# Adamtaranto/frisk

Measured on AMD Instinct MI355X. Metric: windows/sec (k=1..8, w=5kb, s=1kb), higher is better.
Workload: dtype u8/u4 counts + f64 scores

## Files before the change

frisk_amd/csrc/scan8_kernel.h:

```cpp
#pragma once
#include "scan_kernel.h"
#include "ring_rows.h"

#define FRISK8_ORPH_CAP 24
#define FRISK8_UNROLL1 2
#define FRISK8_SHORT_LANES 6
#define FRISK8_PRIO 3
#define FRISK8_RING_PAD 16
#define FRISK8_SLOTS 8

enum { M8_NPLACED = 1,
       M8_PMASK = 3,
       M8_TSUM = 6,
       M8_SAFE = 7 };

template <int KMAX, int BITS, int LOGN, int NT, bool SIDE = false>
struct Lds8 {
    static constexpr uint32_t small = 0;
    static constexpr uint32_t small_bytes = 2736;
    static constexpr uint32_t orphans = small + small_bytes;
    static constexpr uint32_t NL = 1u << (2 * (KMAX - 3));
    static constexpr uint32_t pre = (orphans + FRISK8_ORPH_CAP * 2 + 15) / 16 * 16;
    static constexpr uint32_t side = pre + NL * 12;
    static constexpr uint32_t logtab = side + (SIDE ? 256 : 0);
    static constexpr uint32_t rctab = logtab + uint32_t(LOGN) * 16;
    static constexpr uint32_t misc = rctab + (SIDE ? 256 * 16 : 16 * (BITS == 4 ? 16 : 8));
    static constexpr uint32_t t8 = (misc + 2 * FRISK8_SLOTS * 4 + uint32_t(NT / 64) * 3 * 8 + 15) / 16 * 16;
    static constexpr uint32_t t8_bytes = (1u << (2 * KMAX)) * BITS / 8;
    static constexpr uint32_t total = t8 + t8_bytes;
    static constexpr uint32_t granules = (total + 1279) / 1280;
};

template <int N, int DEG>
__device__ inline double log_tab_n(double x, const double2* tab) {
    const int k = __builtin_amdgcn_frexp_exp(x);
    const double m = __builtin_amdgcn_frexp_mant(x);
    const uint32_t off = (uint32_t(__double2hiint(m)) >> ((N == 128 ? 13 : (N == 64 ? 14 : 15)) - 4)) & (uint32_t(N - 1) << 4);
    const double2 e = *reinterpret_cast<const double2*>(reinterpret_cast<const char*>(tab) + off);
    const double r = __builtin_fma(m, e.x, -1.0);
    double p = (DEG & 1) ? 1.0 / DEG : -1.0 / DEG;
#pragma unroll
    for (int d = DEG - 1; d >= 2; --d) p = __builtin_fma(r, p, (d & 1) ? 1.0 / d : -1.0 / d);
    return __builtin_fma(double(k), 0.69314718055994530942, e.y) + __builtin_fma(r * r, p, r);
}

template <int CTRL>
__device__ inline uint32_t dpp_addu(uint32_t x) {
    return x + uint32_t(__builtin_amdgcn_update_dpp(0, int(x), CTRL, 0xF, 0xF, false));
}
__device__ inline uint32_t wave_sum_u32(uint32_t x) {
    x = dpp_addu<0xB1>(x); x = dpp_addu<0x4E>(x); x = dpp_addu<0x141>(x); x = dpp_addu<0x140>(x);
    return __builtin_amdgcn_readlane(int(x), 0) + __builtin_amdgcn_readlane(int(x), 16) +
           __builtin_amdgcn_readlane(int(x), 32) + __builtin_amdgcn_readlane(int(x), 48);
}

__global__ void scan8_decide_kernel(const unsigned int* __restrict__ counts, unsigned int n_sampled, double side_share, int side_ok,
                                    unsigned int* __restrict__ verdict) {
    const unsigned int handed = counts[0], would = counts[2], scored = counts[3];
    unsigned int form = (double(handed) <= 0.3 * double(n_sampled)) ? 1u : 3u;
    if (form == 1u && side_ok && double(handed + would) > side_share * double(handed + scored)) form = 2u;
    verdict[0] = form; verdict[1] = handed; verdict[2] = would; verdict[3] = scored;
}

template <int KMAX, int NT, int ITS, int BITS, int LOGN, int WPS, bool DEBUG, int ROLE = 0, bool SIDE = false>
__global__ __launch_bounds__(NT, WPS) void scan8_kernel(const ScanParams P) {
    static_assert(KMAX >= 6 && KMAX <= 8, "highest order 6, 7 or 8");
    constexpr int K = KMAX, LVL = KMAX - 3;
    constexpr uint32_t NK = 1u << (2 * K), NL = 1u << (2 * LVL);
    static_assert(BITS == 4 || BITS == 8, "order-8 counters are 4 or 8 bits wide");
    static_assert(LOGN == 32 || LOGN == 64 || LOGN == 128, "logarithm table of 32, 64 or 128 bins");
    constexpr int LOGDEG = LOGN == 128 ? 5 : (LOGN == 64 ? 6 : 7);
    static_assert(ITS + 7 <= 32, "a lane's positions and their max-mers must fit the 32 bases it loads");
    constexpr int NW = NT / 64;
    constexpr int SHW = BITS == 8 ? 2 : 3;
    constexpr uint32_t PERM = (32 / BITS) - 1;
    static_assert(!SIDE || (KMAX == 8 && BITS == 4 && !DEBUG && NT == 256), "the side table exists for the 4-bit form at K = 8");
    using L = Lds8<KMAX, BITS, LOGN, NT, SIDE>;
    constexpr bool CLEAR_ALL = L::t8_bytes / 16 / NT <= uint32_t(ITS);
    constexpr bool FUSED = (KMAX >= 7 && NT >= 256 && NT % 256 == 0);
    constexpr bool PLACE = FUSED && !DEBUG;
    __shared__ __attribute__((aligned(16))) unsigned char lds[L::total];
    const int tid0 = threadIdx.x;
    const int kmin0 = P.kmin;
    uint32_t* t8 = reinterpret_cast<uint32_t*>(lds + L::t8);
    const unsigned char* t8b = lds + L::t8;
    uint32_t* small32 = reinterpret_cast<uint32_t*>(lds + L::small);
    uint16_t* small16 = reinterpret_cast<uint16_t*>(lds + L::small);
    uint16_t* orph = reinterpret_cast<uint16_t*>(lds + L::orphans);
    double* preA = reinterpret_cast<double*>(lds + L::pre);
    uint32_t* preW = reinterpret_cast<uint32_t*>(lds + L::pre + NL * 8);
    uint32_t* side32 = reinterpret_cast<uint32_t*>(lds + L::side);
    const unsigned char* side8 = lds + L::side;
    auto put_pre = [&](uint32_t idx, double A, uint32_t W, uint32_t sd = 0u) __attribute__((always_inline)) {
        if constexpr (SIDE) { preA[idx] = A; preW[idx] = W | (sd << 23); }
        else { preA[idx] = A; preW[idx] = W; }
    };
    auto bump = [&](uint32_t c16, auto sign_c) __attribute__((always_inline)) {
        constexpr int SIGN = decltype(sign_c)::value;
        if (SIDE && ((c16 ^ (c16 >> 8)) & 0xFFu) == 0u) {
            const uint32_t one = 1u << ((c16 & 3u) * 8u);
            if (SIGN > 0) atomicAdd(&side32[(c16 & 0xFFu) >> 2], one); else atomicSub(&side32[(c16 & 0xFFu) >> 2], one);
        } else {
            const uint32_t one = 1u << ((c16 & PERM) * BITS);
            if (SIGN > 0) atomicAdd(&t8[c16 >> SHW], one); else atomicSub(&t8[c16 >> SHW], one);
        }
    };
    uint32_t* misc_base = reinterpret_cast<uint32_t*>(lds + L::misc);
    double* scratch = reinterpret_cast<double*>(lds + L::misc + 2 * FRISK8_SLOTS * 4);
    const double2* logtab = reinterpret_cast<const double2*>(lds + L::logtab);
    double2* rstab = reinterpret_cast<double2*>(lds + L::rctab);
    double* rctab = reinterpret_cast<double*>(lds + L::rctab);

    auto clear_t8 = [&]() {
#pragma unroll
        for (int i = tid0; i < int(L::t8_bytes / 16); i += NT) reinterpret_cast<uint4*>(t8)[i] = make_uint4(0, 0, 0, 0);
        if (SIDE && tid0 < 64) side32[tid0] = 0u;
    };
    auto clear_small = [&]() {
        for (uint32_t i = tid0; i < L::small_bytes / 16; i += NT) reinterpret_cast<uint4*>(small32)[i] = make_uint4(0, 0, 0, 0);
    };
    if (P.in_list != nullptr && *P.in_count == 0u) return;
    if (P.verdict != nullptr && *P.verdict != P.my_form) return;
    __builtin_amdgcn_s_setprio(FRISK8_PRIO);
    clear_t8();
    clear_small();
    if (tid0 < 2 * FRISK8_SLOTS) misc_base[tid0] = 0;
    {
        double2* lt = reinterpret_cast<double2*>(lds + L::logtab);
        for (int i = tid0; i < LOGN; i += NT) lt[i] = reinterpret_cast<const double2*>(LOGN == 128 ? P.log_tab : (LOGN == 64 ? P.log_tab64 : P.log_tab32))[i];
        if constexpr (SIDE) {
            static_assert(!SIDE || NT >= 256, "one thread per entry of the reciprocal table");
            if (tid0 < 256) {
                double r = P.rc_tab[tid0 & 15];
                if (tid0 >= 16) {
                    const double dc = double(tid0);
                    r = __builtin_amdgcn_rcp(dc);
                    r = __builtin_fma(r, __builtin_fma(-dc, r, 1.0), r);
                    r = __builtin_fma(r, __builtin_fma(-dc, r, 1.0), r);
                }
                rstab[tid0] = make_double2(r, 0.0);
            }
        } else if (tid0 < 16) {
            if (BITS == 4) rstab[tid0] = make_double2(P.rc_tab[tid0], 0.0); else rctab[tid0] = P.rc_tab[tid0];
        }
    }
    __syncthreads();

    const int G = gridDim.x;
    int v = blockIdx.x;
    if ((G & 7) == 0) v = (blockIdx.x & 7) * (G >> 3) + (blockIdx.x >> 3);
    const bool listed = P.in_list != nullptr;
    const int64_t chunk = listed ? 1 : P.chunk;
    const int64_t nall = listed ? int64_t(*P.in_count) : (P.c1 - P.c0 + chunk - 1) / chunk;
    const int64_t M = P.sel_mod;
    const int64_t nsample = (nall + M - 1) / M;
    const int64_t nchunks = listed || P.sel_mode == 0 ? nall : (P.sel_mode == 1 ? nsample : nall - nsample);

    ScafDesc d;
    d.cand0 = 0; d.ncand = 0; d.off = 0; d.size = 0; d.kind = 0; d.base0 = 0; d.j0 = 0;
    int dsi = -1;
    uint32_t parity = 0;
    const int slide_pp = P.in_list == nullptr ? P.slide_pp : 0;
    constexpr bool RING = KMAX == 8 && BITS == 4 && !(ROLE & 2);
    char* const ring = RING ? reinterpret_cast<char*>(P.ig_ring) : nullptr;
    const uint32_t slice_off = RING ? uint32_t((size_t(NK) + size_t(blockIdx.x) * (size_t(ITS) * FRISK8_RING_COLS + FRISK8_RING_PAD)) * 8) : 0u;
    bool slide_next = false;
    bool ring_next = false;

    auto window_of = [&](int64_t cand, int64_t& st, int64_t& rep_start, int64_t& rep_stop, int& n, bool& jump) {
        const int64_t j = cand - d.cand0 + d.j0;
        jump = false;
        if (d.kind == 1) { st = 0; n = int(d.size); rep_start = 1; rep_stop = d.size; }
        else {
            st = j * P.inc;
            n = P.w;
            rep_start = st + 1; rep_stop = st + P.w;
            if (st + P.w > d.size) {
                jump = true;
                st = d.size - P.w;
                rep_start = st; rep_stop = d.size;
                if (st < 0) { st += d.size; if (st < 0) st = 0; }
                n = int(d.size - st);
            }
        }
    };
    typedef const __attribute__((address_space(4))) ScanParams* KernargView;
    KernargView Pk = (KernargView)__builtin_amdgcn_kernarg_segment_ptr();
    uint32_t* next_q = reinterpret_cast<uint32_t*>(scratch);
    const bool dealt = Pk->queue != nullptr;
    const uint32_t NQ = dealt ? uint32_t(P.queue_n) : 1u;
    const uint32_t myq = blockIdx.x % NQ;
    uint32_t dry = 0, ahead = 0;
    if (dealt && tid0 == 0) ahead = atomicAdd(&Pk->queue[myq], 1u);
    for (int64_t qs = v;; qs += G) {
        int64_t q = qs;
        asm volatile("" : "+s"(Pk));
        if (dealt) {
            if (tid0 == 0) {
                uint32_t got = 0xFFFFFFFFu;
                while (dry < NQ) {
                    const uint32_t j = (myq + dry) % NQ;
                    const int64_t b = nchunks * j / NQ, len = nchunks * (j + 1) / NQ - b;
                    if (int64_t(ahead) < len) { got = uint32_t(b + ahead); break; }
                    if (++dry < NQ) ahead = atomicAdd(&Pk->queue[(myq + dry) % NQ], 1u);
                }
                *next_q = got;
                if (got != 0xFFFFFFFFu) ahead = atomicAdd(&Pk->queue[(myq + dry) % NQ], 1u);
            }
            __syncthreads();
            const uint32_t got = uint32_t(__builtin_amdgcn_readfirstlane(int(*next_q)));
            __syncthreads();
            if (got == 0xFFFFFFFFu) break;
            q = int64_t(got);
        }
        if (q >= nchunks) break;
        int64_t qq = q;
        if (!listed && P.sel_mode == 1) qq = q * M;
        if (!listed && P.sel_mode == 2) qq = (q / (M - 1)) * M + 1 + q % (M - 1);
        const int64_t cb = listed ? q : P.c0 + qq * chunk;
        const int64_t ce = listed ? q + 1 : ((cb + chunk < P.c1) ? cb + chunk : P.c1);
        for (int64_t ci = cb; ci < ce; ++ci) {
            const int64_t cand = listed ? Pk->in_list[ci] : ci;
            if (cand < d.cand0 || cand >= d.cand0 + d.ncand) {
                int lo = 0, hi = P.n_desc - 1;
                while (lo < hi) {
                    const int mid = (lo + hi + 1) >> 1;
                    if (Pk->descs[mid].cand0 <= cand) lo = mid; else hi = mid - 1;
                }
                d = Pk->descs[lo];
                dsi = lo;
                auto s64 = [](int64_t x) -> int64_t {
                    return int64_t((uint64_t(uint32_t(__builtin_amdgcn_readfirstlane(int(uint64_t(x) >> 32)))) << 32) |
                                   uint32_t(__builtin_amdgcn_readfirstlane(int(uint32_t(uint64_t(x))))));
                };
                d.off = s64(d.off); d.size = s64(d.size); d.cand0 = s64(d.cand0); d.ncand = s64(d.ncand);
                d.base0 = s64(d.base0); d.j0 = s64(d.j0); d.kind = __builtin_amdgcn_readfirstlane(d.kind);
            }
            int tid = tid0, kmin = kmin0;
            asm volatile("" : "+v"(tid), "+s"(kmin));
            asm volatile("" : "+s"(Pk));
            const int lane = tid & 63;
            int64_t st, rep_start, rep_stop;
            int n;
            bool jump = false;
            window_of(cand, st, rep_start, rep_stop, n, jump);
            const int64_t g0 = d.off + (st - d.base0);
            const int64_t row = cand - P.c0;
            const uint32_t ring_base = RING ? uint32_t(uint64_t(st) % uint64_t(ITS * FRISK8_RING_COLS)) : 0u;
            const uint32_t rb_q = ring_base / uint32_t(ITS), rb_r = ring_base - rb_q * uint32_t(ITS);
            const uint32_t lane_col0 = RING ? ring_lane_col(rb_q, uint32_t(tid), 0u) : 0u;
            const uint32_t lane_col1 = RING ? ring_lane_col(rb_q, uint32_t(tid), 1u) : 0u;
            auto ring_uni = [&](int it) __attribute__((always_inline)) -> uint32_t {
                return ring_uni_general<ITS>(slice_off, rb_r, it);
            };
            auto ring_lane = [&](int it) __attribute__((always_inline)) -> uint32_t {
                return ring_lane_general<ITS>(rb_r, it, lane_col0, lane_col1);
            };
            auto ring_mine = [&](int it) __attribute__((always_inline)) -> uint32_t { return ring_uni(it) + ring_lane(it); };
            constexpr bool ROWS = RING && ITS == 20;
            typedef const __attribute__((address_space(1))) char* GlobalBytes;
            typedef const __attribute__((address_space(1))) double* GlobalDouble;
            GlobalBytes row0_base = ROWS ? (GlobalBytes)(ring + slice_off + ring_row0_base_row(0) * FRISK8_RING_ROW_BYTES) : nullptr;
            const uint32_t row0_lane = ROWS ? ring_off_row0(slice_off, rb_q, uint32_t(tid), 0) : 0u;
            const bool sliding = slide_next;
            const bool lane_new = !sliding || !ring_next || tid * ITS + (ITS - 1) >= P.w - (K - 1) - P.inc;
            ring_next = false;
            slide_next = slide_pp > 0 && ci + 1 < ce && d.kind == 0 && !jump && cand + 1 < d.cand0 + d.ncand &&
                         st + int64_t(P.inc) + P.w <= d.size;
            if (n > NT * ITS) {
                if (tid == 0) { const unsigned int slot = atomicAdd(Pk->out_count, 1u); Pk->out_list[slot] = cand; }
                continue;
            }
            uint32_t* misc = misc_base + parity * FRISK8_SLOTS;
            uint32_t* misc_other = misc_base + (parity ^ 1u) * FRISK8_SLOTS;
            parity ^= 1u;

            const int j0 = tid * ITS;
            const int64_t gl = g0 + (j0 < n ? j0 : 0);
            const int64_t wi = gl >> 4, mi = gl >> 5;
            const int shc = 32 - int(gl & 15) * 2, shm = 32 - int(gl & 31);
            const uint32_t w0 = P.codes[wi], w1 = P.codes[wi + 1], w2 = P.codes[wi + 2];
            const uint32_t i0 = P.inv[mi], i1 = P.inv[mi + 1], l0 = P.low[mi], l1 = P.low[mi + 1];
            uint64_t scode = 0, ecode = 0;
            uint32_t sfull = 0, efull = 0;
            if (sliding) {
                const int q0 = tid * slide_pp;
                const int cnt = P.inc - q0;
                const int64_t gs = g0 - P.inc + (cnt > 0 ? q0 : 0);
                const int64_t ge = g0 + (P.w - (K - 1) - P.inc) + (cnt > 0 ? q0 : 0);
                const int64_t swi = gs >> 4, smi = gs >> 5, ewi = ge >> 4, emi = ge >> 5;
                const uint32_t s0 = P.codes[swi], s1 = P.codes[swi + 1], s2 = P.codes[swi + 2], si0 = P.inv[smi], si1 = P.inv[smi + 1];
                const uint32_t e0 = P.codes[ewi], e1 = P.codes[ewi + 1], e2 = P.codes[ewi + 2], ei0 = P.inv[emi], ei1 = P.inv[emi + 1];
                auto funnel = [](uint32_t a, uint32_t b, uint32_t c, int sh) -> uint64_t {
                    return (uint64_t(uint32_t(((uint64_t(a) << 32) | b) >> sh)) << 32) | uint32_t(((uint64_t(b) << 32) | c) >> sh);
                };
                auto starts = [](uint32_t inv32, int cnt_, int pp) -> uint32_t {
                    uint32_t f = ~inv32;
                    f &= f << 1; f &= f << 2;
                    f &= f << (K - 4);
                    const int m = cnt_ < pp ? cnt_ : pp;
                    return m > 0 ? f & uint32_t(0xFFFFFFFF00000000ull >> m) : 0u;
                };
                scode = funnel(s0, s1, s2, 32 - int(gs & 15) * 2);
                ecode = funnel(e0, e1, e2, 32 - int(ge & 15) * 2);
                sfull = starts(uint32_t(((uint64_t(si0) << 32) | si1) >> (32 - int(gs & 31))), cnt, slide_pp);
                efull = starts(uint32_t(((uint64_t(ei0) << 32) | ei1) >> (32 - int(ge & 31))), cnt, slide_pp);
            }
            const uint32_t chi = uint32_t(((uint64_t(w0) << 32) | w1) >> shc);
            const uint32_t clo = uint32_t(((uint64_t(w1) << 32) | w2) >> shc);
            const uint64_t acode = (uint64_t(chi) << 32) | clo;
            const uint32_t ainv = uint32_t(((uint64_t(i0) << 32) | i1) >> shm);
            const uint32_t alow = uint32_t(((uint64_t(l0) << 32) | l1) >> shm);
            auto topbits = [](int k) -> uint32_t {
                k = k < 0 ? 0 : (k > 32 ? 32 : k);
                return uint32_t(0xFFFFFFFF00000000ull >> k);
            };
            constexpr uint32_t MINE = uint32_t(0xFFFFFFFF00000000ull >> ITS);
            const int nleft = n - j0;
            const uint32_t actm = topbits(nleft) & MINE;
            const uint32_t vld = ~ainv;
            uint32_t fullm = vld;
            fullm &= fullm << 1; fullm &= fullm << 2;
            fullm &= fullm << (K - 4);
            fullm &= topbits(nleft - (K - 1)) & MINE;
            auto code_at = [&](int it) -> uint32_t { return uint32_t(acode >> (64 - 2 * K - 2 * it)) & (NK - 1u); };
            {
                uint32_t cAll = 0, cGC = 0, nvalid = 0;
                auto gc_plane = [&]() -> uint32_t {
                    auto squeeze = [](uint32_t w) -> uint32_t {
                        uint32_t x = (w >> 1) & 0x55555555u;
                        x = (x | (x >> 1)) & 0x33333333u;
                        x = (x | (x >> 2)) & 0x0F0F0F0Fu;
                        x = (x | (x >> 4)) & 0x00FF00FFu;
                        x = (x | (x >> 8)) & 0x0000FFFFu;
                        return x;
                    };
                    return (squeeze(uint32_t(acode >> 32)) << 16) | squeeze(uint32_t(acode));
                };
                auto tally = [&](uint32_t sel, uint32_t ntop_) {
                    static_assert(ITS <= 31, "three ten-bit fields: a lane's counts below 32, a pair of rows' sums below 1024");
                    uint32_t gcl;
                    if (__any(sel != actm)) gcl = uint32_t(__popc(sel & gc_plane()));
                    else gcl = uint32_t(__popcll(acode & 0xAAAAAAAAAAAAAAAAull & ~(0xFFFFFFFFFFFFFFFFull >> (2 * __popc(actm)))));
                    uint32_t x = uint32_t(__popc(sel)) | (gcl << 10) | (ntop_ << 20);
                    x = dpp_addu<0xB1>(x); x = dpp_addu<0x4E>(x); x = dpp_addu<0x141>(x); x = dpp_addu<0x140>(x);
                    const uint32_t a = uint32_t(__builtin_amdgcn_readlane(int(x), 0) + __builtin_amdgcn_readlane(int(x), 16));
                    const uint32_t b = uint32_t(__builtin_amdgcn_readlane(int(x), 32) + __builtin_amdgcn_readlane(int(x), 48));
                    cAll = (a & 1023u) + (b & 1023u);
                    cGC = ((a >> 10) & 1023u) + ((b >> 10) & 1023u);
                    nvalid = (a >> 20) + (b >> 20);
                };
                auto short_word = [&](uint32_t c16, uint32_t inv8, int rem) {
                    int run = lead_clear8(inv8);
                    run = run < rem ? run : rem;
                    run = run < K ? run : K - 1;
                    const int rs = run < LVL ? run : LVL;
                    if (rs >= kmin && !(PLACE && run >= K - 2)) {
                        const uint32_t b = uint32_t(table_offset(kmin, rs)) + (c16 >> (2 * K - 2 * rs));
                        atomicAdd(&small32[b >> 1], 1u << ((b & 1u) * 16));
                    }
                    if (run >= K - 2) {
                        const uint32_t slot = atomicAdd(&misc[M_NORPH], 1u);
                        if (slot < FRISK8_ORPH_CAP)
                            orph[slot] = uint16_t(run == K - 1 ? (c16 >> 2) : (0x8000u | ((c16 >> 4) << 2)));
                    }
                };
                const uint32_t shortm = actm & ~fullm;
                const unsigned long long short_lanes = __ballot(shortm != 0u);
                const bool few = __popcll(short_lanes) <= FRISK8_SHORT_LANES;
                if (!sliding) {
#pragma unroll FRISK8_UNROLL1
                    for (int it = 0; it < ITS; ++it) {
                        const uint32_t bit = 0x80000000u >> it;
                        const uint32_t c16 = code_at(it);
                        if (fullm & bit) bump(c16, std::integral_constant<int, 1>{});
                        else if (!few && (shortm & bit)) short_word(c16, (ainv >> (24 - it)) & 0xFFu, n - (j0 + it));
                    }
                } else {
#pragma unroll 2
                    for (int it = 0; it < slide_pp; ++it) {
                        const uint32_t bit = 0x80000000u >> it;
                        const uint32_t cs = uint32_t(scode >> (64 - 2 * K - 2 * it)) & (NK - 1u);
                        const uint32_t cn = uint32_t(ecode >> (64 - 2 * K - 2 * it)) & (NK - 1u);
                        if (sfull & bit) bump(cs, std::integral_constant<int, -1>{});
                        if (efull & bit) bump(cn, std::integral_constant<int, 1>{});
                    }
                    if (!few) {
                        for (int it = 0; it < ITS; ++it)
                            if (shortm & (0x80000000u >> it)) short_word(code_at(it), (ainv >> (24 - it)) & 0xFFu, n - (j0 + it));
                    }
                }
                if (few) {
                    for (unsigned long long rest = short_lanes; rest; rest &= rest - 1) {
                        const int src = int(__ffsll((long long)rest)) - 1;
                        const uint32_t sm = uint32_t(__builtin_amdgcn_readlane(int(shortm), src));
                        const uint32_t si = uint32_t(__builtin_amdgcn_readlane(int(ainv), src));
                        const uint32_t sh = uint32_t(__builtin_amdgcn_readlane(int(uint32_t(acode >> 32)), src));
                        const uint32_t sl = uint32_t(__builtin_amdgcn_readlane(int(uint32_t(acode)), src));
                        const int sleft = __builtin_amdgcn_readlane(nleft, src);
                        const int it = lane < ITS ? lane : 0;
                        if (lane < ITS && ((sm >> (31 - it)) & 1u)) {
                            const uint64_t sc = (uint64_t(sh) << 32) | sl;
                            short_word(uint32_t(sc >> (64 - 2 * K - 2 * it)) & (NK - 1u), (si >> (24 - it)) & 0xFFu, sleft - it);
                        }
                    }
                }
                tally(actm & vld & ~alow, uint32_t(__popc(fullm)));
                {
                    const unsigned long long have = __ballot(fullm != 0u);
                    if (have) {
                        const uint32_t mine = uint32_t(acode >> (64 - 2 * K - 2 * int(__clz(int(fullm | 1u))))) & (NK - 1u);
                        const uint32_t pick = uint32_t(__builtin_amdgcn_readlane(int(mine), int(__ffsll((long long)have)) - 1));
                        if (lane == 0) misc[M8_SAFE] = pick;
                    }
                }
                if (lane == 0) {
                    if (cAll) atomicAdd(&misc[M_UPA], cAll);
                    if (cGC) atomicAdd(&misc[M_UPG], cGC);
                    if (nvalid) atomicAdd(&misc[M_NVALID], nvalid);
                }
            }
            __syncthreads();
            if (tid < FRISK8_SLOTS) misc_other[tid] = 0;

            const uint32_t o5 = uint32_t(table_offset(kmin, LVL));
            if constexpr (!FUSED) {
                uint32_t tot = 0;
                for (uint32_t q5 = tid; q5 < NL; q5 += NT) {
                    uint32_t s = 0;
                    if (BITS == 8) {
#pragma unroll
                        for (int m = 0; m < 4; ++m) {
                            const uint32_t mm = (uint32_t(m) + (uint32_t(tid) >> 2)) & 3u;
                            const uint4 x = *reinterpret_cast<const uint4*>(t8b + q5 * 64u + mm * 16u);
                            s = __builtin_amdgcn_sad_u8(x.x, 0u, s); s = __builtin_amdgcn_sad_u8(x.y, 0u, s);
                            s = __builtin_amdgcn_sad_u8(x.z, 0u, s); s = __builtin_amdgcn_sad_u8(x.w, 0u, s);
                        }
                    } else {
#pragma unroll
                        for (int m = 0; m < 2; ++m) {
                            const uint32_t mm = (uint32_t(m) + (uint32_t(tid) >> 3)) & 1u;
                            const uint4 x = *reinterpret_cast<const uint4*>(t8b + q5 * 32u + mm * 16u);
                            s = __builtin_amdgcn_udot8(x.x, 0x11111111u, s, false); s = __builtin_amdgcn_udot8(x.y, 0x11111111u, s, false);
                            s = __builtin_amdgcn_udot8(x.z, 0x11111111u, s, false); s = __builtin_amdgcn_udot8(x.w, 0x11111111u, s, false);
                        }
                    }
                    tot += s;
                    small16[o5 + q5] = uint16_t(small16[o5 + q5] + s);
                }
                tot = wave_sum_u32(tot);
                if (lane == 0 && tot) atomicAdd(&misc[M8_TSUM], tot);
                __syncthreads();
            }
            if constexpr (LVL == 3) {
                if (tid < 64 && kmin <= 2) {
                    const uint32_t c3 = small16[uint32_t(table_offset(kmin, 3)) + uint32_t(tid)];
                    uint32_t qs = dpp_addu<0xB1>(c3);
                    qs = dpp_addu<0x4E>(qs);
                    const uint32_t o2 = uint32_t(table_offset(kmin, 2));
                    uint32_t c2 = 0;
                    if ((tid & 3) == 0) { c2 = small16[o2 + (tid >> 2)] + qs; small16[o2 + (tid >> 2)] = uint16_t(c2); }
                    if (kmin <= 1) {
                        uint32_t rs = dpp_addu<0xB1>(c2);
                        rs = dpp_addu<0x4E>(rs); rs = dpp_addu<0x141>(rs); rs = dpp_addu<0x140>(rs);
                        if ((tid & 15) == 0) small16[tid >> 4] = uint16_t(small16[tid >> 4] + rs);
                    }
                }
                __syncthreads();
            }

            auto uni = [](uint32_t x) -> uint32_t { return __builtin_amdgcn_readfirstlane(x); };
            const uint32_t upAll = uni(misc[M_UPA]), upGC = uni(misc[M_UPG]);
            const int64_t S = int64_t(upAll);
            const int64_t nn = n - S;
            const bool keep = !(double(nn) >= 0.3 * double(n));
            uint32_t status = (jump ? ROW_JUMPBACK : 0u);
            const uint32_t nvalid_top = uni(misc[M_NVALID]);
            const int n_orph = int(uni(misc[M_NORPH]));
            const bool wrapped = (!FUSED && uni(misc[M8_TSUM]) != nvalid_top) || n_orph > FRISK8_ORPH_CAP;
            const uint32_t safe_code = uni(misc[M8_SAFE]);

            auto zero_own = [&]() {
#pragma unroll 4
                for (int it = 0; it < ITS; ++it)
                    if (fullm & (0x80000000u >> it)) t8[code_at(it) >> SHW] = 0u;
            };
            auto hand_over = [&]() {
                if (!slide_next) clear_t8();
                clear_small();
                if (tid == 0) { const unsigned int slot = atomicAdd(Pk->out_count, 1u); Pk->out_list[slot] = cand; }
                __syncthreads();
            };
            if (wrapped) { hand_over(); continue; }
            if (!keep) {
                if (!slide_next) { if (CLEAR_ALL) clear_t8(); else zero_own(); }
                clear_small();
                if (tid == 0) {
                    Pk->seq_index[row] = dsi; Pk->start[row] = rep_start; Pk->stop[row] = rep_stop;
                    Pk->status[row] = status;
                    const double qnan = __longlong_as_double(0x7FF8000000000000LL);
                    Pk->kld[row] = qnan; Pk->gc[row] = qnan;
                    if (P.flags & 1u) { Pk->pi[row] = qnan; Pk->si[row] = qnan; Pk->cri[row] = qnan; }
                    if (DEBUG && P.dbg_meta) {
                        P.dbg_meta[row * 3 + 0] = n; P.dbg_meta[row * 3 + 1] = 0; P.dbg_meta[row * 3 + 2] = nn;
                    }
                }
                __syncthreads();
                continue;
            }
            if (tid == 0) { Pk->seq_index[row] = dsi; Pk->start[row] = rep_start; Pk->stop[row] = rep_stop; }

            uint32_t o6[4] = {0xFFFFFFFFu, 0xFFFFFFFFu, 0xFFFFFFFFu, 0xFFFFFFFFu}, o7[4] = {0xFFFFFFFFu, 0xFFFFFFFFu, 0xFFFFFFFFu, 0xFFFFFFFFu};
            uint32_t o7c[4] = {0xFFFFFFFFu, 0xFFFFFFFFu, 0xFFFFFFFFu, 0xFFFFFFFFu};
            int n7 = 0, n_list = 0;
            uint32_t rest_mask = 0;
            static_assert(L::orphans % 8 == 0 && FRISK8_ORPH_CAP <= 31, "the orphan list: eight-byte aligned, one mask bit per entry (bit 31 of the mask word: SIDE)");
            auto load_orphans = [&](uint32_t placed) {
                uint32_t todo = (n_orph >= 32 ? 0xFFFFFFFFu : ((1u << n_orph) - 1u)) & ~placed;
                n_list = __popc(todo);
#pragma unroll
                for (int k = 0; k < 4; ++k) {
                    if (todo) {
                        const int j = __ffs(int(todo)) - 1;
                        todo &= todo - 1u;
                        const uint32_t e = uni(orph[j]);
                        o6[k] = (e >> 2) & (NK / 16u - 1u);
                        if (!(e & 0x8000u)) o7[k] = e;
                    }
                }
                rest_mask = todo;
#pragma unroll
                for (int k = 0; k < 4; ++k) {
                    if (o7[k] != 0xFFFFFFFFu) {
#pragma unroll
                        for (int q = 0; q < 4; ++q) if (q == n7) o7c[q] = o7[k];
                        ++n7;
                    }
                }
            };
            struct Fetched { double Ig, A5; uint32_t W5, c8, w7, roff; uint4 w6; };
            auto fetch = [&](uint32_t c16, int it = 0, int mode = 0) __attribute__((always_inline)) -> Fetched {
                Fetched f;
                f.roff = 0;
                if constexpr (RING) {
                    f.Ig = 1.0;
                    if (mode == 3) {
                        if (ring_row0_steps(it)) {
                            row0_base += (ring_row0_base_row(it) - ring_row0_base_row(it - 1)) * FRISK8_RING_ROW_BYTES;
                            asm volatile("" : "+s"(row0_base));
                        }
                        f.Ig = *(GlobalDouble)((row0_base + lane_col0) + ring_row0_imm(it));
                    } else if (mode == 4) {
                        f.roff = ring_row0_from_lane(row0_lane, it);
                        f.Ig = *reinterpret_cast<const double*>(ring + (lane_new ? (c16 << 3) : f.roff));
                    } else if (mode) {
                        f.roff = ring_mine(it);
                        if (mode == 1)
                            f.Ig = *reinterpret_cast<const double*>((ring + ring_uni(it)) + ring_lane(it));
                        else
                            f.Ig = *reinterpret_cast<const double*>(ring + ((mode == 2 && lane_new) ? (c16 << 3) : f.roff));
                    }
                } else {
                f.Ig = *reinterpret_cast<const double*>(reinterpret_cast<const char*>(P.ig) + (c16 << 3));
                }
                if (BITS == 8) {
                    f.c8 = t8b[c16];
                    f.w7 = *reinterpret_cast<const uint32_t*>(t8b + (c16 & ~3u));
                    f.w6 = *reinterpret_cast<const uint4*>(t8b + (c16 & ~15u));
                } else {
                    f.c8 = 0;
                    f.w7 = 0;
                    const uint2 x = *reinterpret_cast<const uint2*>(t8b + ((c16 >> 4) << 3));
                    f.w6 = make_uint4(x.x, x.y, 0u, 0u);
                }
                f.W5 = *reinterpret_cast<const uint32_t*>(lds + L::pre + NL * 8 + ((c16 >> 6) << 2));
                f.A5 = *reinterpret_cast<const double*>(lds + L::pre + ((c16 >> 6) << 3));
                return f;
            };
            auto table_counts = [&](const Fetched& f, uint32_t c16, uint32_t& c8, uint32_t& c7, uint32_t& c6, uint32_t tper = 0xFFFFFFFFu) __attribute__((always_inline)) {
                if (BITS == 8) {
                    c8 = f.c8;
                    c7 = __builtin_amdgcn_sad_u8(f.w7, 0u, 0u);
                    c6 = __builtin_amdgcn_sad_u8(f.w6.x, 0u, __builtin_amdgcn_sad_u8(f.w6.y, 0u, __builtin_amdgcn_sad_u8(f.w6.z, 0u, __builtin_amdgcn_sad_u8(f.w6.w, 0u, 0u))));
                } else {
                    const uint32_t w7 = uint32_t(((uint64_t(f.w6.y) << 32) | f.w6.x) >> ((c16 & 12u) << 2));
                    uint32_t s6 = 0u, s7 = 0u, s8 = 0u;
                    if constexpr (SIDE) {
                        const uint32_t t = tper != 0xFFFFFFFFu ? tper : ((c16 ^ (c16 >> 8)) & 0xFFu);
                        const uint32_t sd = f.W5 >> 23;
                        s6 = t < 16u ? sd : 0u; s7 = t < 4u ? sd : 0u; s8 = t == 0u ? sd : 0u;
                    }
                    c8 = __builtin_amdgcn_ubfe(w7, (c16 & 3u) * 4u, 4u) + s8;
                    c7 = __builtin_amdgcn_udot8(w7, 0x1111u, s7, false);
                    c6 = __builtin_amdgcn_udot8(f.w6.x, 0x11111111u, __builtin_amdgcn_udot8(f.w6.y, 0x11111111u, s6, false), false);
                }
            };
            auto add_orphans = [&](uint32_t c16, uint32_t& c7, uint32_t& c6) __attribute__((always_inline)) {
                const uint32_t q6 = c16 >> 4, q7 = c16 >> 2;
#pragma unroll
                for (int k = 0; k < 4; ++k) {
                    c7 += (q7 == o7[k]) ? 1u : 0u;
                    c6 += (q6 == o6[k]) ? 1u : 0u;
                }
                for (uint32_t m = rest_mask; m; m &= m - 1u) {
                    const uint32_t e = orph[__ffs(int(m)) - 1];
                    c7 += (q7 == e) ? 1u : 0u;
                    c6 += (q6 == ((e >> 2) & (NK / 16u - 1u))) ? 1u : 0u;
                }
            };
            auto count = [&](int x, uint32_t c) -> uint32_t {
                if (x <= LVL) return small16[table_offset(kmin, x) + c];
                uint32_t c8, c7, c6;
                const uint32_t c16 = c << (2 * (K - x));
                table_counts(fetch(c16), c16, c8, c7, c6);
                add_orphans(c16, c7, c6);
                return x == K ? c8 : (x == K - 1 ? c7 : c6);
            };
            uint32_t pend0 = 0xFFFFFFFFu, pend1 = 0xFFFFFFFFu;
            double r_lane = 0.0;
            if (lane <= 8) r_lane = div_exact(double(1u << (2 * lane)), double(int32_t((S - (lane - 1)) * 2)));
            auto r_of = [&](int x) -> double {
                return __hiloint2double(__builtin_amdgcn_readlane(__double2hiint(r_lane), x),
                                        __builtin_amdgcn_readlane(__double2loint(r_lane), x));
            };
            if (BITS == 4 && (SIDE || tid < 16)) rstab[tid & 255].y = double(uint32_t((tid & 255) * (tid & 255))) * r_of(K);
            {
                constexpr int LV = LVL;
                double rx[LV + 1];
                uint32_t ox[LV + 1], wm[LV + 1];
#pragma unroll
                for (int x = 1; x <= LV; ++x) {
                    const bool on = x >= kmin;
                    rx[x] = on ? r_of(x) : 0.0;
                    ox[x] = on ? uint32_t(table_offset(kmin, x)) : 0u;
                    wm[x] = on ? 0xFFFFFFFFu : 0u;
                }
                if constexpr (LV >= 4) {
                    static_assert(NT >= 256 && NT % 64 == 0, "thread t <-> 4-mer t: the first four waves (the others sit this stage out)");
                    if (NT == 256 || tid < 256) {
                    const uint32_t q4 = uint32_t(tid);
                    uint64_t extra = 0;
                    if constexpr (PLACE) {
                        pend0 = 0xFFFFFFFFu; pend1 = 0xFFFFFFFFu;
                        for (int k = 0; k < n_orph; ++k) {
                            const uint32_t e = orph[k];
                            const uint32_t q6 = (e >> 2) & (NK / 16u - 1u);
                            if ((q6 >> (2 * (K - 2) - 8)) != q4) continue;
                            uint32_t slot = 0xFFFFFFFFu;
                            if constexpr (BITS == 4) {
                                const uint2 g = *reinterpret_cast<const uint2*>(t8b + q6 * 8u);
                                if (!(e & 0x8000u)) {
                                    const uint32_t f = ((e & 2u) ? g.y : g.x) >> ((e & 1u) * 16u) & 0xFFFFu;
                                    uint32_t z = ~(f | (f >> 1) | (f >> 2) | (f >> 3)) & 0x1111u;
                                    if (SIDE && ((e ^ (e >> 8)) & 0x3Fu) == 0u) z &= ~(1u << (((e >> 6) & 3u) * 4u));
                                    if (z) slot = ((e & 0x3FFFu) << 2) | uint32_t((__ffs(int(z)) - 1) >> 2);
                                } else {
                                    uint32_t zz = ((g.x & 0xFFFFu) == 0u ? 1u : 0u) | ((g.x >> 16) == 0u ? 2u : 0u) |
                                                  ((g.y & 0xFFFFu) == 0u ? 4u : 0u) | ((g.y >> 16) == 0u ? 8u : 0u);
                                    if (SIDE && ((q6 ^ (q6 >> 8)) & 0xFu) == 0u) zz &= ~(1u << ((q6 >> 6) & 3u));
                                    if (zz) slot = ((q6 << 2) | uint32_t(__ffs(int(zz)) - 1)) << 2;
                                }
                            } else {
                                const uint4 g = *reinterpret_cast<const uint4*>(t8b + q6 * 16u);
                                if (!(e & 0x8000u)) {
                                    const uint32_t sub = e & 3u;
                                    const uint32_t f = sub == 0u ? g.x : (sub == 1u ? g.y : (sub == 2u ? g.z : g.w));
                                    const uint32_t z = (f - 0x01010101u) & ~f & 0x80808080u;
                                    if (z) slot = ((e & 0x3FFFu) << 2) | uint32_t((__ffs(int(z)) - 1) >> 3);
                                } else {
                                    const uint32_t zz = (g.x == 0u ? 1u : 0u) | (g.y == 0u ? 2u : 0u) | (g.z == 0u ? 4u : 0u) | (g.w == 0u ? 8u : 0u);
                                    if (zz) slot = ((q6 << 2) | uint32_t(__ffs(int(zz)) - 1)) << 2;
                                }
                            }
                            if (slot != 0xFFFFFFFFu && pend1 == 0xFFFFFFFFu) {
                                atomicAdd(&t8[slot >> SHW], 1u << ((slot & PERM) * BITS));
                                if (pend0 == 0xFFFFFFFFu) pend0 = (uint32_t(k) << 16) | slot; else pend1 = (uint32_t(k) << 16) | slot;
                                atomicOr(&misc[M8_PMASK], 1u << k);
                                atomicAdd(&misc[M8_NPLACED], 1u);
                            } else {
                                extra += K == 8 ? (1ull << (16u * ((q6 >> 2) & 3u))) : 1ull;
                            }
                        }
                    }
                    uint32_t c5[4] = {0u, 0u, 0u, 0u}, j5[4] = {0u, 1u, 2u, 3u};
                    uint32_t side_mine = 0;
                    if constexpr (LV == 5) {
                        const uint2 ch = *reinterpret_cast<const uint2*>(small16 + ox[5] + 4 * q4);
                        if constexpr (FUSED) {
                            if constexpr (SIDE) { side_mine = side8[q4]; extra += uint64_t(side_mine) << (16u * (q4 >> 6)); }
                            const uint64_t d64 = ((uint64_t(ch.y) << 32) | ch.x) + extra;
                            const unsigned char* mine = t8b + q4 * (BITS == 8 ? 256u : 128u);
                            constexpr int NH = BITS == 8 ? 4 : 2;
                            uint4 x[4][NH];
#pragma unroll
                            for (int m = 0; m < 4; ++m) {
                                const uint32_t j = (uint32_t(m) + uint32_t(tid)) & 3u;
#pragma unroll
                                for (int h = 0; h < NH; ++h) {
                                    const uint32_t hh = BITS == 8 ? ((uint32_t(h) + (uint32_t(tid) >> 1)) & 3u) : ((uint32_t(h) + (uint32_t(tid) >> 2)) & 1u);
                                    x[m][h] = *reinterpret_cast<const uint4*>(mine + j * (BITS == 8 ? 64u : 32u) + hh * 16u);
                                }
                            }
                            uint32_t tot = side_mine;
#pragma unroll
                            for (int m = 0; m < 4; ++m) {
                                const uint32_t j = (uint32_t(m) + uint32_t(tid)) & 3u;
                                uint32_t sm = 0;
#pragma unroll
                                for (int h = 0; h < NH; ++h) {
                                    if (BITS == 8) {
                                        sm = __builtin_amdgcn_sad_u8(x[m][h].x, 0u, sm); sm = __builtin_amdgcn_sad_u8(x[m][h].y, 0u, sm);
                                        sm = __builtin_amdgcn_sad_u8(x[m][h].z, 0u, sm); sm = __builtin_amdgcn_sad_u8(x[m][h].w, 0u, sm);
                                    } else {
                                        sm = __builtin_amdgcn_udot8(x[m][h].x, 0x11111111u, sm, false); sm = __builtin_amdgcn_udot8(x[m][h].y, 0x11111111u, sm, false);
                                        sm = __builtin_amdgcn_udot8(x[m][h].z, 0x11111111u, sm, false); sm = __builtin_amdgcn_udot8(x[m][h].w, 0x11111111u, sm, false);
                                    }
                                }
                                tot += sm;
                                j5[m] = j;
                                c5[m] = sm + (uint32_t(d64 >> (16u * j)) & 0xFFFFu);
                                if (DEBUG) small16[ox[5] + 4 * q4 + j] = uint16_t(c5[m]);
                            }
                            tot = wave_sum_u32(tot);
                            if (lane == 0 && tot) atomicAdd(&misc[M8_TSUM], tot);
                        } else {
                            c5[0] = ch.x & 0xFFFFu; c5[1] = ch.x >> 16; c5[2] = ch.y & 0xFFFFu; c5[3] = ch.y >> 16;
                        }
                    }
                    uint32_t cx[5] = {0u, 0u, 0u, 0u, 0u};
                    uint32_t below4 = 0;
                    if constexpr (LV == 4 && FUSED) {
                        const unsigned char* mine = t8b + q4 * 64u;
                        uint4 x[4];
#pragma unroll
                        for (int h = 0; h < 4; ++h) x[h] = *reinterpret_cast<const uint4*>(mine + ((uint32_t(h) + (uint32_t(tid) >> 1)) & 3u) * 16u);
#pragma unroll
                        for (int h = 0; h < 4; ++h) {
                            below4 = __builtin_amdgcn_sad_u8(x[h].x, 0u, below4); below4 = __builtin_amdgcn_sad_u8(x[h].y, 0u, below4);
                            below4 = __builtin_amdgcn_sad_u8(x[h].z, 0u, below4); below4 = __builtin_amdgcn_sad_u8(x[h].w, 0u, below4);
                        }
                        const uint32_t tot = wave_sum_u32(below4);
                        if (lane == 0 && tot) atomicAdd(&misc[M8_TSUM], tot);
                    }
                    const uint32_t d4 = small16[ox[4] + q4], d3 = small16[ox[3] + (q4 >> 2)], d2 = small16[ox[2] + (q4 >> 4)], d1 = small16[q4 >> 6];
                    if (kmin <= 4) {
                        cx[4] = d4 + below4 + (LV == 4 ? uint32_t(extra) : 0u);
                        if constexpr (LV == 4 && FUSED) small16[ox[4] + q4] = uint16_t(cx[4]);
                        if constexpr (LV == 5) {
                            cx[4] += c5[0] + c5[1] + c5[2] + c5[3];
                            small16[ox[4] + q4] = uint16_t(cx[4]);
                        }
                        if (kmin <= 3) {
                            uint32_t qs = dpp_addu<0xB1>(cx[4]);
                            qs = dpp_addu<0x4E>(qs);
                            cx[3] = d3 + qs;
                            if ((lane & 3) == 0) small16[ox[3] + (q4 >> 2)] = uint16_t(cx[3]);
                            if (kmin <= 2) {
                                uint32_t rs = dpp_addu<0xB1>((lane & 3) == 0 ? cx[3] : 0u);
                                rs = dpp_addu<0x4E>(rs); rs = dpp_addu<0x141>(rs); rs = dpp_addu<0x140>(rs);
                                cx[2] = d2 + rs;
                                if ((lane & 15) == 0) small16[ox[2] + (q4 >> 4)] = uint16_t(cx[2]);
                                if (kmin <= 1) {
                                    const uint32_t ws = __builtin_amdgcn_readlane(int(cx[2]), 0) + __builtin_amdgcn_readlane(int(cx[2]), 16) +
                                                        __builtin_amdgcn_readlane(int(cx[2]), 32) + __builtin_amdgcn_readlane(int(cx[2]), 48);
                                    cx[1] = d1 + ws;
                                    if (lane == 0) small16[q4 >> 6] = uint16_t(cx[1]);
                                }
                            }
                        }
                    }
                    uint32_t W4 = 0;
                    double A4 = 0.0;
#pragma unroll
                    for (int x = 1; x <= 4; ++x) {
                        const double cd = double(cx[x]);
                        W4 += (cx[x] & wm[x]) << (2 * x);
                        A4 = __builtin_fma(cd * cd, rx[x], A4);
                    }
                    if constexpr (LV == 4) {
                        put_pre(q4, A4, W4);
                    } else {
                        double A5[4];
                        uint32_t W5[4];
#pragma unroll
                        for (int m = 0; m < 4; ++m) {
                            const double cd = double(c5[m]);
                            W5[m] = W4 + ((c5[m] & wm[5]) << 10);
                            A5[m] = __builtin_fma(cd * cd, rx[5], A4);
                        }
                        if constexpr (FUSED) {
#pragma unroll
                            for (int m = 0; m < 4; ++m) put_pre(4 * q4 + j5[m], A5[m], W5[m], side_mine);
                            if (SIDE && (ROLE & 1) && side_mine >= 16u) atomicOr(&misc[M8_PMASK], 0x80000000u);
                        } else {
                            auto lo = [](double x) -> uint32_t { return uint32_t(__double2loint(x)); };
                            auto hi = [](double x) -> uint32_t { return uint32_t(__double2hiint(x)); };
                            uint4* oa = reinterpret_cast<uint4*>(preA + 4 * q4);
                            oa[0] = make_uint4(lo(A5[0]), hi(A5[0]), lo(A5[1]), hi(A5[1]));
                            oa[1] = make_uint4(lo(A5[2]), hi(A5[2]), lo(A5[3]), hi(A5[3]));
                            *reinterpret_cast<uint4*>(preW + 4 * q4) = make_uint4(W5[0], W5[1], W5[2], W5[3]);
                        }
                    }
                    }
                } else {
#pragma unroll 2
                    for (uint32_t c = tid; c < NL; c += NT) {
                        uint32_t cx[LV + 1];
#pragma unroll
                        for (int x = 1; x <= LV; ++x) cx[x] = small16[ox[x] + (c >> (2 * (LV - x)))];
                        uint32_t W = 0;
                        double A = 0.0;
#pragma unroll
                        for (int x = 1; x <= LV; ++x) {
                            const double cd = double(cx[x]);
                            W += (cx[x] & wm[x]) << (2 * x);
                            A = __builtin_fma(cd * cd, rx[x], A);
                        }
                        put_pre(c, A, W);
                    }
                }
            }
            __syncthreads();
            const uint32_t pmask_raw = PLACE ? uni(misc[M8_PMASK]) : 0u;
            const uint32_t placed = pmask_raw & 0x7FFFFFFFu;
            if constexpr (PLACE) {
                if (pend0 != 0xFFFFFFFFu) orph[pend0 >> 16] = uint16_t(pend0);
                if (pend1 != 0xFFFFFFFFu) orph[pend1 >> 16] = uint16_t(pend1);
            }
            auto remove_fakes = [&]() {
                if (PLACE && placed && tid < FRISK8_ORPH_CAP && ((placed >> tid) & 1u) && (slide_next || !CLEAR_ALL)) {
                    const uint32_t slot = orph[tid];
                    if (slide_next) atomicSub(&t8[slot >> SHW], 1u << ((slot & PERM) * BITS));
                    else t8[slot >> SHW] = 0u;
                }
            };
            if constexpr (FUSED) {
                if (uni(misc[M8_TSUM]) != nvalid_top + (PLACE ? uni(misc[M8_NPLACED]) : 0u)) {
                    if (PLACE && placed) __syncthreads();
                    remove_fakes(); hand_over(); continue;
                }
            }
            if (SIDE && (ROLE & 1) && tid == 0) { atomicAdd(Pk->out_count + 3, 1u); if (pmask_raw >> 31) atomicAdd(Pk->out_count + 2, 1u); }
            load_orphans(placed);

            if (DEBUG && P.dbg_counts) {
                uint32_t* out = P.dbg_counts + row * int64_t(P.nprof);
                for (int x = kmin; x <= K; ++x) {
                    const int64_t off = table_offset(kmin, x);
                    for (uint32_t c = tid; c < (1u << (2 * x)); c += NT) out[off + c] = count(x, c);
                }
            }
            if (DEBUG && P.dbg_meta && tid == 0) {
                P.dbg_meta[row * 3 + 0] = n;
                P.dbg_meta[row * 3 + 1] = (n >= K ? n - K + 1 : 0) - int64_t(nvalid_top);
                P.dbg_meta[row * 3 + 2] = nn;
            }
            if (nvalid_top == 0) status |= ROW_NO_MAXMER;
            if (nvalid_top > 0 && S >= kmin - 1 && S <= K - 1) status |= ROW_ZERO_WEIGHT;
            status |= ROW_KEPT;
            if (tid == 0) {
                Pk->gc[row] = __longlong_as_double((long long)((uint64_t(uint32_t(S)) << 32) | upGC));
                if (P.flags & 1u) {
                    const double qnan = __longlong_as_double(0x7FF8000000000000LL);
                    const uint32_t AT = count(2, 1), TA = count(2, 4), TG = count(2, 6), GT = count(2, 9), CA = count(2, 12), AC = count(2, 3);
                    const double pi = AT > 0 ? double(TA) / double(AT) : qnan;
                    const double si = (AC + GT) > 0 ? double(CA + TG) / double(AC + GT) : qnan;
                    Pk->pi[row] = pi;
                    Pk->si[row] = si;
                    Pk->cri[row] = (pi == 0.0 || si == 0.0) ? qnan : pi - si;
                }
            }

            const double r6 = r_of(K - 2), r7 = r_of(K - 1), r8 = r_of(K);
            double sw = 0.0, sg = 0.0, stt = 0.0;
            __builtin_amdgcn_s_setprio(0);
            auto shl_add = [](uint32_t a, auto sh, uint32_t b) __attribute__((always_inline)) -> uint32_t {
                uint32_t r;
                asm("v_lshl_add_u32 %0, %1, %2, %3" : "=v"(r) : "v"(a), "n"(decltype(sh)::value), "v"(b));
                return r;
            };
            auto score_one = [&](const Fetched& f, uint32_t c8, uint32_t c7, uint32_t c6, uint32_t sel, bool on)
                                 __attribute__((always_inline)) {
                double2 rs;
                if constexpr (BITS == 4) rs = rstab[sel & (SIDE ? 255u : 15u)];
                else {
                    rs = make_double2(rctab[sel & 15u], double(__umul24(sel, sel)) * r8);
                    if (__builtin_expect(__any(c8 >= 16u), 0)) {
                        if (on && c8 >= 16u) {
                            const double dc = double(c8);
                            double r = __builtin_amdgcn_rcp(dc);
                            r = __builtin_fma(r, __builtin_fma(-dc, r, 1.0), r);
                            r = __builtin_fma(r, __builtin_fma(-dc, r, 1.0), r);
                            rs.x = r;
                        }
                    }
                }
                const uint32_t W = shl_add(c8, std::integral_constant<int, 2 * K>{},
                                           shl_add(c7, std::integral_constant<int, 2 * K - 2>{},
                                                   shl_add(c6, std::integral_constant<int, 2 * K - 4>{}, SIDE ? (f.W5 & 0x7FFFFFu) : f.W5)));
                double A = __builtin_fma(double(__umul24(c6, c6)), r6, f.A5);
                A = __builtin_fma(double(__umul24(c7, c7)), r7, A);
                A = A + rs.y;
                const double den = double(W) * f.Ig;
                double rr = __builtin_amdgcn_rcp(den);
                rr = __builtin_fma(rr, __builtin_fma(-den, rr, 1.0), rr);
                const double ratio = A * rr;
                const double Igr = f.Ig * rs.x;
                const double Iwr = ratio * Igr;
                const double ln = log_tab_n<LOGN, LOGDEG>(ratio, logtab);
                sw += Iwr;
                sg += Igr;
                stt = __builtin_fma(Iwr, ln, stt);
            };
            uint32_t ah = uint32_t(acode >> 32), al = uint32_t(acode), fm4 = fullm;
            asm volatile("" : "+v"(ah), "+v"(al), "+v"(fm4));
            const uint64_t acode4 = (uint64_t(ah) << 32) | al;
            auto raw4_at = [&](int it) -> uint32_t { return uint32_t(acode4 >> (64 - 2 * K - 2 * it)) & (NK - 1u); };
            const uint64_t aper = SIDE ? (acode4 ^ (acode4 >> 8)) : 0ull;
            auto per4_at = [&](int it) -> uint32_t { return SIDE ? (uint32_t(aper >> (64 - 2 * K - 2 * it)) & 0xFFu) : 0xFFFFFFFFu; };
            constexpr int GR = (K == 8 && BITS == 4 && !SIDE) ? 2 : 1;
            constexpr bool ROLLED = K < 8 || NT > 256;
            auto score_all = [&](auto allon_c, auto orph_c, auto park_c, auto row0_c) __attribute__((always_inline)) {
                constexpr bool ALLON = decltype(allon_c)::value;
                constexpr bool PARK = RING && decltype(park_c)::value;
                constexpr bool ROW0 = ROWS && decltype(row0_c)::value;
                constexpr int FMODE = (PARK ? 2 : 1) + (ROW0 ? 2 : 0);
                static_assert(!(ROW0 && ROLLED), "the row-aligned ring access needs the unrolled scoring loop");
                constexpr int ORPH = decltype(orph_c)::value;
                auto on_at = [&](int it) -> bool { return ALLON || ((fm4 >> (31 - it)) & 1u); };
                auto code4_at = [&](int it) -> uint32_t {
                    return on_at(it) ? raw4_at(it) : safe_code;
                };
                auto score_group = [&](Fetched (&f)[GR], int g, auto check_c) __attribute__((always_inline)) {
                    constexpr bool CHECK = decltype(check_c)::value;
                    uint32_t c8[GR], c7[GR], c6[GR];
#pragma unroll
                    for (int k = 0; k < GR; ++k) {
                        if (!CHECK || g + k < ITS) table_counts(f[k], code4_at(g + k), c8[k], c7[k], c6[k], per4_at(g + k));
                    }
#pragma unroll
                    for (int k = 0; k < GR; ++k) {
                        if (!CHECK || g + k < ITS) {
                            const uint32_t c16 = code4_at(g + k), q6 = c16 >> 4, q7 = c16 >> 2;
                            constexpr int N6 = ORPH == -1 ? 0 : (ORPH == 2 ? 2 : 4), N7 = ORPH == -1 ? 0 : (ORPH == 2 ? 1 : 4);
#pragma unroll
                            for (int j = 0; j < N7; ++j) c7[k] += (q7 == o7c[j]) ? 1u : 0u;
#pragma unroll
                            for (int j = 0; j < N6; ++j) c6[k] += (q6 == o6[j]) ? 1u : 0u;
                            if (ORPH == 0)
                                for (uint32_t m = rest_mask; m; m &= m - 1u) {
                                    const uint32_t e = orph[__ffs(int(m)) - 1];
                                    c7[k] += (q7 == e) ? 1u : 0u;
                                    c6[k] += (q6 == ((e >> 2) & (NK / 16u - 1u))) ? 1u : 0u;
                                }
                        }
                    }
#pragma unroll
                    for (int k = 0; k < GR; ++k) {
                        if (!CHECK || g + k < ITS) {
                            if constexpr (PARK) *reinterpret_cast<double*>(ring + f[k].roff) = on_at(g + k) ? f[k].Ig : 1.0;
                            score_one(f[k], c8[k], c7[k], c6[k], on_at(g + k) ? c8[k] : 0u, on_at(g + k));
                        }
                    }
                };
                if constexpr (ROLLED && ITS % (2 * GR) == 0) {
                    Fetched bufA[GR], bufB[GR];
#pragma unroll
                    for (int k = 0; k < GR; ++k) bufA[k] = fetch(code4_at(k), k, FMODE);
#pragma unroll 1
                    for (int g = 0; g < ITS; g += 2 * GR) {
#pragma unroll
                        for (int k = 0; k < GR; ++k) bufB[k] = fetch(code4_at(g + GR + k), g + GR + k, FMODE);
                        score_group(bufA, g, std::false_type{});
                        __builtin_amdgcn_sched_barrier(0);
                        const int gn = g + 2 * GR < ITS ? g + 2 * GR : 0;
#pragma unroll
                        for (int k = 0; k < GR; ++k) bufA[k] = fetch(code4_at(gn + k), gn + k, FMODE);
                        score_group(bufB, g + GR, std::false_type{});
                        __builtin_amdgcn_sched_barrier(0);
                    }
                    return;
                }
                Fetched buf[2][GR];
#pragma unroll
                for (int k = 0; k < GR; ++k) if (k < ITS) buf[0][k] = fetch(code4_at(k), k, FMODE);
#pragma unroll
                for (int g = 0; g < ITS; g += GR) {
                    const int cur = (g / GR) & 1;
#pragma unroll
                    for (int k = 0; k < GR; ++k) if (g + GR + k < ITS) buf[cur ^ 1][k] = fetch(code4_at(g + GR + k), g + GR + k, FMODE);
                    score_group(buf[cur], g, std::true_type{});
                    __builtin_amdgcn_sched_barrier(0);
                }
            };
            constexpr uint32_t ALL_MINE = uint32_t(0xFFFFFFFF00000000ull >> ITS);
            using orphX = std::integral_constant<int, -1>;
            using orph2 = std::integral_constant<int, 2>;
            using orph4 = std::integral_constant<int, 4>;
            using orphN = std::integral_constant<int, 0>;
            const bool wave_parks = RING && __any(lane_new);
            using yes = std::true_type;
            using no = std::false_type;
            if constexpr (PLACE) {
                if (n_list == 0) {
                    auto hot = [&](auto allon_c, auto park_c) __attribute__((always_inline)) {
                        if constexpr (ROWS) {
                            if (rb_r == 0u) { score_all(allon_c, orphX{}, park_c, yes{}); return; }
                        }
                        score_all(allon_c, orphX{}, park_c, no{});
                    };
                    if (__all(fm4 == ALL_MINE)) { if (wave_parks) hot(yes{}, yes{}); else hot(yes{}, no{}); }
                    else { if (wave_parks) hot(no{}, yes{}); else hot(no{}, no{}); }
                } else if (n_list <= 4) score_all(no{}, orph4{}, yes{}, no{});
                else score_all(no{}, orphN{}, yes{}, no{});
            } else {
                if (n_list <= 2 && n7 <= 1) {
                    if (__all(fm4 == ALL_MINE)) score_all(yes{}, orph2{}, yes{}, no{});
                    else score_all(no{}, orph2{}, yes{}, no{});
                } else if (n_list <= 4) score_all(no{}, orph4{}, yes{}, no{});
                else score_all(no{}, orphN{}, yes{}, no{});
            }

            __builtin_amdgcn_s_setprio(FRISK8_PRIO);
            sw = wave_sum_exact(sw); sg = wave_sum_exact(sg); stt = wave_sum_exact(stt);
            if (lane == 0) { double* p = scratch + (tid >> 6) * 3; p[0] = sw; p[1] = sg; p[2] = stt; }
            __syncthreads();
            ring_next = true;
            remove_fakes();
            if (!slide_next) {
                if constexpr (CLEAR_ALL) clear_t8();
                else {
#pragma unroll 4
                    for (int it = 0; it < ITS; ++it)
                        if (fm4 & (0x80000000u >> it)) t8[raw4_at(it) >> SHW] = 0u;
                }
            }
            clear_small();
            if (tid == 0) {
                double a = 0.0, b = 0.0, c = 0.0;
                for (int w = 0; w < NW; ++w) { a += scratch[3 * w]; b += scratch[3 * w + 1]; c += scratch[3 * w + 2]; }
                Pk->status[row] = status;
                Pk->sw[row] = a;
                Pk->sg[row] = b;
                Pk->kld[row] = c;
            }
            __syncthreads();
        }
    }
}
```

Measured before the change: 65.63 million.

## Add tail-lane classification so end-of-sequence waves take the row-aligned scoring path

Lanes at the sequence tail, whose k-mer starts are clipped by the end of the sequence, are classified into full, clamped or last classes. The class is stored in the two free low bits of the lane mask. When every lane in a wave has a known class and the ring row is aligned, the wave runs a new specialised scoring copy with uniform code streams and per-class count masks, in place of the generic per-lane predicated path. This adds a kernel instantiation and extra mask logic, which may raise code size and register pressure, and it only matters for waves near sequence ends.

Result: no change. 66.26 million, median of 6 (+1.0%).

```diff
diff --git a/frisk_amd/csrc/scan8_kernel.h b/frisk_amd/csrc/scan8_kernel.h
--- a/frisk_amd/csrc/scan8_kernel.h
+++ b/frisk_amd/csrc/scan8_kernel.h
@@ -1,6 +1,7 @@
 #pragma once
 #include "scan_kernel.h"
 #include "ring_rows.h"
+#include "tail_lanes.h"
 
 #define FRISK8_ORPH_CAP 24
 #define FRISK8_UNROLL1 2
@@ -322,7 +323,11 @@
             uint32_t fullm = vld;
             fullm &= fullm << 1; fullm &= fullm << 2;
             fullm &= fullm << (K - 4);
+            const uint32_t uncut = fullm & MINE;
             fullm &= topbits(nleft - (K - 1)) & MINE;
+            constexpr bool TAILS = ROWS && PLACE && K == 8 && NT == 256;
+            uint32_t fmc = fullm;
+            if constexpr (TAILS) fmc |= tail_lane_class<ITS, K>(fullm, uncut, nleft, n);
             auto code_at = [&](int it) -> uint32_t { return uint32_t(acode >> (64 - 2 * K - 2 * it)) & (NK - 1u); };
             {
                 uint32_t cAll = 0, cGC = 0, nvalid = 0;
@@ -912,7 +917,7 @@
                 sg += Igr;
                 stt = __builtin_fma(Iwr, ln, stt);
             };
-            uint32_t ah = uint32_t(acode >> 32), al = uint32_t(acode), fm4 = fullm;
+            uint32_t ah = uint32_t(acode >> 32), al = uint32_t(acode), fm4 = fmc;
             asm volatile("" : "+v"(ah), "+v"(al), "+v"(fm4));
             const uint64_t acode4 = (uint64_t(ah) << 32) | al;
             auto raw4_at = [&](int it) -> uint32_t { return uint32_t(acode4 >> (64 - 2 * K - 2 * it)) & (NK - 1u); };
@@ -920,15 +925,22 @@
             auto per4_at = [&](int it) -> uint32_t { return SIDE ? (uint32_t(aper >> (64 - 2 * K - 2 * it)) & 0xFFu) : 0xFFFFFFFFu; };
             constexpr int GR = (K == 8 && BITS == 4 && !SIDE) ? 2 : 1;
             constexpr bool ROLLED = K < 8 || NT > 256;
-            auto score_all = [&](auto allon_c, auto orph_c, auto park_c, auto row0_c) __attribute__((always_inline)) {
+            auto score_all = [&](auto allon_c, auto orph_c, auto park_c, auto row0_c, auto tail_c) __attribute__((always_inline)) {
                 constexpr bool ALLON = decltype(allon_c)::value;
                 constexpr bool PARK = RING && decltype(park_c)::value;
                 constexpr bool ROW0 = ROWS && decltype(row0_c)::value;
+                constexpr bool TAIL = TAILS && decltype(tail_c)::value;
+                static_assert(!TAIL || (!ALLON && PARK && ROW0 && decltype(orph_c)::value == -1), "the tail copy: row-aligned, parking, no orphans on the list");
+                constexpr int NLO = ITS - (K - 1);
+                const uint32_t cls = TAIL ? (fm4 & 3u) : 0u;
+                const uint32_t m_lo = TAIL ? tail_m_lo(cls) : 0u, m_hi = TAIL ? tail_m_hi(cls) : 0u;
+                const uint64_t acodeT = TAIL ? tail_stream<K>(cls, acode4) : 0ull;
                 constexpr int FMODE = (PARK ? 2 : 1) + (ROW0 ? 2 : 0);
                 static_assert(!(ROW0 && ROLLED), "the row-aligned ring access needs the unrolled scoring loop");
                 constexpr int ORPH = decltype(orph_c)::value;
                 auto on_at = [&](int it) -> bool { return ALLON || ((fm4 >> (31 - it)) & 1u); };
                 auto code4_at = [&](int it) -> uint32_t {
+                    if constexpr (TAIL) return it < NLO ? raw4_at(it) : tail_code_from<K>(acodeT, it);
                     return on_at(it) ? raw4_at(it) : safe_code;
                 };
                 auto score_group = [&](Fetched (&f)[GR], int g, auto check_c) __attribute__((always_inline)) {
@@ -958,6 +970,11 @@
 #pragma unroll
                     for (int k = 0; k < GR; ++k) {
                         if (!CHECK || g + k < ITS) {
+                            if constexpr (TAIL) {
+                                *reinterpret_cast<double*>(ring + f[k].roff) = f[k].Ig;
+                                score_one(f[k], c8[k], c7[k], c6[k], c8[k] & (g + k < NLO ? m_lo : m_hi), true);
+                                continue;
+                            }
                             if constexpr (PARK) *reinterpret_cast<double*>(ring + f[k].roff) = on_at(g + k) ? f[k].Ig : 1.0;
                             score_one(f[k], c8[k], c7[k], c6[k], on_at(g + k) ? c8[k] : 0u, on_at(g + k));
                         }
@@ -1005,20 +1022,21 @@
                 if (n_list == 0) {
                     auto hot = [&](auto allon_c, auto park_c) __attribute__((always_inline)) {
                         if constexpr (ROWS) {
-                            if (rb_r == 0u) { score_all(allon_c, orphX{}, park_c, yes{}); return; }
-                        }
-                        score_all(allon_c, orphX{}, park_c, no{});
+                            if (rb_r == 0u) { score_all(allon_c, orphX{}, park_c, yes{}, no{}); return; }
+                        }
+                        score_all(allon_c, orphX{}, park_c, no{}, no{});
                     };
-                    if (__all(fm4 == ALL_MINE)) { if (wave_parks) hot(yes{}, yes{}); else hot(yes{}, no{}); }
+                    if (__all(fm4 == (ALL_MINE | (TAILS ? TAIL_FULL : 0u)))) { if (wave_parks) hot(yes{}, yes{}); else hot(yes{}, no{}); }
+                    else if (TAILS && wave_parks && rb_r == 0u && __all((fm4 & 3u) != TAIL_NONE)) score_all(no{}, orphX{}, yes{}, yes{}, yes{});
                     else { if (wave_parks) hot(no{}, yes{}); else hot(no{}, no{}); }
-                } else if (n_list <= 4) score_all(no{}, orph4{}, yes{}, no{});
-                else score_all(no{}, orphN{}, yes{}, no{});
+                } else if (n_list <= 4) score_all(no{}, orph4{}, yes{}, no{}, no{});
+                else score_all(no{}, orphN{}, yes{}, no{}, no{});
             } else {
                 if (n_list <= 2 && n7 <= 1) {
-                    if (__all(fm4 == ALL_MINE)) score_all(yes{}, orph2{}, yes{}, no{});
-                    else score_all(no{}, orph2{}, yes{}, no{});
-                } else if (n_list <= 4) score_all(no{}, orph4{}, yes{}, no{});
-                else score_all(no{}, orphN{}, yes{}, no{});
+                    if (__all(fm4 == ALL_MINE)) score_all(yes{}, orph2{}, yes{}, no{}, no{});
+                    else score_all(no{}, orph2{}, yes{}, no{}, no{});
+                } else if (n_list <= 4) score_all(no{}, orph4{}, yes{}, no{}, no{});
+                else score_all(no{}, orphN{}, yes{}, no{}, no{});
             }
 
             __builtin_amdgcn_s_setprio(FRISK8_PRIO);
diff --git a/frisk_amd/csrc/tail_lanes.h b/frisk_amd/csrc/tail_lanes.h
--- /dev/null
+++ b/frisk_amd/csrc/tail_lanes.h
@@ -0,0 +1,40 @@
+#pragma once
+
+#include <cstdint>
+
+#if defined(__HIPCC__)
+#define FRISK_TAIL_FN __host__ __device__ inline
+#else
+#define FRISK_TAIL_FN inline
+#endif
+
+enum : uint32_t { TAIL_NONE = 0u, TAIL_FULL = 1u, TAIL_CLAMPED = 2u, TAIL_LAST = 3u };
+
+template <int ITS>
+FRISK_TAIL_FN constexpr uint32_t tail_mine() { return uint32_t(0xFFFFFFFF00000000ull >> ITS); }
+template <int ITS, int K>
+FRISK_TAIL_FN constexpr uint32_t tail_last_starts() { return uint32_t(0xFFFFFFFF00000000ull >> (ITS - (K - 1))); }
+
+template <int ITS, int K>
+FRISK_TAIL_FN uint32_t tail_lane_class(uint32_t fm, uint32_t uncut, int nleft, int n) {
+    static_assert(ITS >= K && ITS <= 30, "a lane holds a max-mer start, and its mask leaves two bits free");
+    if (fm == tail_mine<ITS>()) return TAIL_FULL;
+    if (nleft <= 0 && uncut == tail_mine<ITS>() && n >= ITS + K - 1) return TAIL_CLAMPED;
+    if (nleft == ITS && fm == tail_last_starts<ITS, K>()) return TAIL_LAST;
+    return TAIL_NONE;
+}
+
+FRISK_TAIL_FN uint32_t tail_m_lo(uint32_t cls) { return cls == TAIL_CLAMPED ? 0u : 0xFFFFFFFFu; }
+FRISK_TAIL_FN uint32_t tail_m_hi(uint32_t cls) { return cls == TAIL_FULL ? 0xFFFFFFFFu : 0u; }
+template <int K>
+FRISK_TAIL_FN uint64_t tail_stream(uint32_t cls, uint64_t acode) { return cls == TAIL_FULL ? acode : acode >> (2 * (K - 1)); }
+template <int ITS, int K>
+FRISK_TAIL_FN uint32_t tail_mask_at(uint32_t cls, int it) { return it < ITS - (K - 1) ? tail_m_lo(cls) : tail_m_hi(cls); }
+template <int K>
+FRISK_TAIL_FN uint32_t tail_code_from(uint64_t stream, int it) { return uint32_t(stream >> (64 - 2 * K - 2 * it)) & ((1u << (2 * K)) - 1u); }
+template <int ITS, int K>
+FRISK_TAIL_FN uint32_t tail_code_at(uint32_t cls, uint64_t acode, int it) {
+    return tail_code_from<K>(it < ITS - (K - 1) ? acode : tail_stream<K>(cls, acode), it);
+}
+template <int ITS, int K>
+FRISK_TAIL_FN int tail_code_pos(uint32_t cls, int it) { return (it < ITS - (K - 1) || cls == TAIL_FULL) ? it : it - (K - 1); }
```
